# jhtonyKoo/music_mixing_style_transfer

Hardware: AMD Instinct MI355X
Metric: stereo 44.1 kHz segments/sec (FXencoder+MixFXcloner fwd) (higher is better)
Workload: dtype bf16

## Files before the change

### include/mst_hip.h

```cpp
#ifndef MST_HIP_H
#define MST_HIP_H

#include <stddef.h>
#include <stdint.h>

#ifdef __cplusplus
extern "C" {
#endif

typedef enum {
    MST_OK = 0,
    MST_ERR_ARG = -1,
    MST_ERR_UNSUPPORTED = -2,
    MST_ERR_HIP = -3,
    MST_ERR_STATE = -4,
    MST_ERR_WORKSPACE = -5
} MstStatus;

typedef enum {
    MST_PREC_F32 = 0,
    MST_PREC_BF16 = 1,
    MST_PREC_BF16X3 = 2
} MstPrecision;

#define MST_MAX_BLOCKS 32

int mst_version(void);
const char *mst_last_error(void);

typedef struct MstTcn MstTcn;

typedef struct {
    int nblocks;
    int ninputs;
    int noutputs;
    int channels;
    int kernel_size;
    int cond_dim;
    int dilations[MST_MAX_BLOCKS];
    int causal;
} MstTcnDesc;

int mst_tcn_create(const MstTcnDesc *desc, MstTcn **out);
int mst_tcn_destroy(MstTcn *tcn);

int mst_tcn_load_block(MstTcn *tcn, int n, const float *conv_w, const float *bn_weight, const float *bn_bias,
                       const float *bn_mean, const float *bn_var, float bn_eps, const float *film_w,
                       const float *film_b, const float *res_w, void *stream);
int mst_tcn_load_output(MstTcn *tcn, const float *w, const float *b, void *stream);

int mst_tcn_set_cond(MstTcn *tcn, const float *cond_dev, int n_rows, long block_stride, void *stream);

size_t mst_tcn_workspace_bytes(const MstTcn *tcn, int B, int L, int precision);

int mst_tcn_forward(MstTcn *tcn, const float *x_dev, float *y_dev, int B, int L, int precision,
                    void *workspace, size_t workspace_bytes, void *stream);
int mst_tcn_forward_blocks(MstTcn *tcn, const float *x_dev, float *act_dev, int B, int L, int precision, int n_run,
                           void *workspace, size_t workspace_bytes, void *stream);

int mst_tcn_set_tuning(MstTcn *tcn, int flags);
int mst_tcn_get_tuning(const MstTcn *tcn, int *flags, int *last_forward_fused_block0);

int mst_tcn_set_fusion(MstTcn *tcn, int flags);
int mst_tcn_get_fusion(const MstTcn *tcn, int *flags, int *last_forward_fused_tail);

int mst_tcn_context(const MstTcn *tcn, long *left, long *right);

int mst_tcn_timing_begin(MstTcn *tcn, int max_forwards);
int mst_tcn_timing_end(MstTcn *tcn, float *ms_out, int *n_forwards);

int mst_calib_mainloop(int launches, float *ms_per_launch, float *sclk_mhz, void *stream);

typedef struct MstEnc MstEnc;

typedef struct {
    int nblocks;
    int channels[MST_MAX_BLOCKS + 1];
    int kernels[MST_MAX_BLOCKS];
    int strides[MST_MAX_BLOCKS];
    int dilations[MST_MAX_BLOCKS];
    int valid_padding;
    float act_slope;
} MstEncDesc;

int mst_enc_create(const MstEncDesc *desc, MstEnc **out);
int mst_enc_destroy(MstEnc *enc);
int mst_enc_load_conv(MstEnc *enc, int block, int which, const float *w, const float *bias,
                      const float *bn_weight, const float *bn_bias, const float *bn_mean, const float *bn_var,
                      float bn_eps, void *stream);
int mst_enc_set_tuning(MstEnc *enc, long rows_min_tiles);
int mst_enc_set_schedule(MstEnc *enc, int flags);
int mst_global_avgpool(const float *x_dev, float *y_dev, long rows, int L, void *stream);
int mst_enc_zero_stuff(const float *x_dev, float *y_dev, long rows, long L, int stride, long pad_left, long Lu, void *stream);
size_t mst_enc_workspace_bytes(const MstEnc *enc, int B, int L);
int mst_enc_forward(MstEnc *enc, const float *x_dev, float *emb_dev, int B, int L, int precision, void *workspace,
                    size_t workspace_bytes, void *stream);
int mst_enc_forward_blocks(MstEnc *enc, const float *x_dev, float *out_dev, int B, int L, int precision, int n_run,
                           void *workspace, size_t workspace_bytes, void *stream);
int mst_enc_conv_length(const MstEnc *enc, int block, int which, int L);
int mst_enc_forward_conv(MstEnc *enc, int block, int which, const float *x_dev, float *y_dev, int B, int L, void *stream);
int mst_enc_block_length(const MstEnc *enc, int block, int L);

int mst_film_forward(const float *w_dev, const float *b_dev, const float *cond_dev, int rows, int cond_dim, int C,
                     const float *x_dev, float *y_dev, int B, long L, float *table_dev, void *stream);

int mst_embedding_mean(const float *emb_dev, int n_rows, int dim, float *out_dev, void *stream);

#define MST_SUMSQ_SLOTS 64
#define MST_FX_FORM_EQ_LANE_APPLY 1
#define MST_FX_FORM_EQ_VALU_ENDS 2
#define MST_FX_FORM_COMP_SLICE_SMALL 4
typedef struct {
    unsigned struct_size;
    int forms;
    const double *in_scale_dev;
    double *out_sumsq_dev;
    const double *in_sumsq_dev;
// ... 175 lines not shown
```

### music_mixing_style_transfer_amd/_lib.py

```python
import ctypes as C
import os

import torch

_HERE = os.path.dirname(os.path.abspath(__file__))
LIB_PATH = os.path.join(_HERE, "csrc", "libmst_hip.so")

MST_OK = 0
MST_PREC_F32 = 0
MST_PREC_BF16 = 1
MST_PREC_BF16X3 = 2
MST_MAX_BLOCKS = 32
TCN_TUNING_DEFAULT = 245
TCN_FUSION_DEFAULT = 1
PRECISIONS = {"fp32": MST_PREC_F32, "f32": MST_PREC_F32, "bf16": MST_PREC_BF16, "bf16x3": MST_PREC_BF16X3}

STATUS_NAMES = {0: "MST_OK", -1: "MST_ERR_ARG", -2: "MST_ERR_UNSUPPORTED", -3: "MST_ERR_HIP", -4: "MST_ERR_STATE",
                -5: "MST_ERR_WORKSPACE"}


class MstTcnDesc(C.Structure):
    _fields_ = [("nblocks", C.c_int), ("ninputs", C.c_int), ("noutputs", C.c_int), ("channels", C.c_int),
                ("kernel_size", C.c_int), ("cond_dim", C.c_int), ("dilations", C.c_int * MST_MAX_BLOCKS), ("causal", C.c_int)]


FX_FORM_EQ_LANE_APPLY, FX_FORM_EQ_VALU_ENDS, FX_FORM_COMP_SLICE_SMALL = 1, 2, 4


class MstFxFuse(C.Structure):
    _fields_ = [("struct_size", C.c_uint), ("forms", C.c_int), ("in_scale_dev", C.c_void_p), ("out_sumsq_dev", C.c_void_p),
                ("in_sumsq_dev", C.c_void_p), ("post_rms", C.c_int), ("post_gain", C.c_float), ("out_in_sumsq_dev", C.c_void_p),
                ("out_ms_dev", C.c_void_p), ("in_ms_dev", C.c_void_p)]

    def __init__(self, in_scale_dev=None, out_sumsq_dev=None, in_sumsq_dev=None, post_rms=0, post_gain=0.0, out_in_sumsq_dev=None,
                 out_ms_dev=None, in_ms_dev=None, forms=0):
        super().__init__(C.sizeof(MstFxFuse), forms, in_scale_dev, out_sumsq_dev, in_sumsq_dev, post_rms, post_gain, out_in_sumsq_dev,
                         out_ms_dev, in_ms_dev)


FX_COMP_SPLIT_SERIAL, FX_COMP_TIME_PARALLEL, FX_COMP_WAVE_SERIAL = 0, 1, 2


class MstFxBiquadItemsPlan(C.Structure):
    _fields_ = [("struct_size", C.c_uint), ("M", C.c_int), ("tables_offset", C.c_size_t), ("item_stride", C.c_size_t), ("powers_offset", C.c_size_t),
                ("coef_offset", C.c_size_t), ("total_bytes", C.c_size_t)]

    def __init__(self, *a, **kw):
        super().__init__(*a, **kw)
        self.struct_size = C.sizeof(MstFxBiquadItemsPlan)


class MstFxBiquadPlan(C.Structure):
    _fields_ = [("struct_size", C.c_uint), ("time_parallel", C.c_int), ("M", C.c_int), ("scan_threads", C.c_int), ("record_doubles", C.c_int),
                ("nchunks", C.c_long), ("ends_offset", C.c_size_t), ("starts_offset", C.c_size_t)]

    def __init__(self):
        super().__init__(C.sizeof(MstFxBiquadPlan))


class MstFxCompressorPlan(C.Structure):
    _fields_ = [("struct_size", C.c_uint), ("form", C.c_int), ("nslices", C.c_int), ("record_doubles", C.c_int), ("nchunks", C.c_long),
                ("nbatch", C.c_long), ("ntiles", C.c_long), ("kappa", C.c_double), ("kappa_limit", C.c_double), ("xl_offset", C.c_size_t),
                ("maps_offset", C.c_size_t), ("ystart_offset", C.c_size_t), ("tab_offset", C.c_size_t), ("carry_offset", C.c_size_t),
                ("tsums_offset", C.c_size_t), ("total_bytes", C.c_size_t)]

    def __init__(self):
        super().__init__(C.sizeof(MstFxCompressorPlan))


class MstEncDesc(C.Structure):
    _fields_ = [("nblocks", C.c_int), ("channels", C.c_int * (MST_MAX_BLOCKS + 1)), ("kernels", C.c_int * MST_MAX_BLOCKS),
                ("strides", C.c_int * MST_MAX_BLOCKS), ("dilations", C.c_int * MST_MAX_BLOCKS), ("valid_padding", C.c_int), ("act_slope", C.c_float)]


MST_MSS_MAX_SCALES = 8
MSS_MODES = {"midside": 0, "ori": 1}
MSS_WINDOWS = {"hann": 0, "hamming": 1}


class MstMssDesc(C.Structure):
    _fields_ = [("struct_size", C.c_uint), ("mode", C.c_int), ("n_scales", C.c_int), ("n_fft", C.c_int * MST_MSS_MAX_SCALES),
                ("hop", C.c_int * MST_MSS_MAX_SCALES), ("win_length", C.c_int * MST_MSS_MAX_SCALES), ("window", C.c_int),
                ("eps", C.c_double)]

    def __init__(self, mode=0, n_fft=(), hop=(), win_length=(), window=0, eps=1e-7):
        super().__init__()
        self.struct_size, self.mode, self.n_scales, self.window, self.eps = C.sizeof(MstMssDesc), mode, len(n_fft), window, eps
        for i in range(min(len(n_fft), MST_MSS_MAX_SCALES)):
            self.n_fft[i], self.hop[i], self.win_length[i] = n_fft[i], hop[i], win_length[i]


_P = C.c_void_p
_F = C.c_void_p

SIGNATURES = {
    "mst_version": (C.c_int, []),
    "mst_last_error": (C.c_char_p, []),
    "mst_tcn_create": (C.c_int, [C.POINTER(MstTcnDesc), C.POINTER(_P)]),
    "mst_tcn_destroy": (C.c_int, [_P]),
    "mst_tcn_load_block": (C.c_int, [_P, C.c_int, _F, _F, _F, _F, _F, C.c_float, _F, _F, _F, _P]),
    "mst_tcn_load_output": (C.c_int, [_P, _F, _F, _P]),
    "mst_tcn_set_cond": (C.c_int, [_P, _F, C.c_int, C.c_long, _P]),
    "mst_tcn_workspace_bytes": (C.c_size_t, [_P, C.c_int, C.c_int, C.c_int]),
    "mst_tcn_forward": (C.c_int, [_P, _F, _F, C.c_int, C.c_int, C.c_int, _P, C.c_size_t, _P]),
    "mst_tcn_forward_blocks": (C.c_int, [_P, _F, _F, C.c_int, C.c_int, C.c_int, C.c_int, _P, C.c_size_t, _P]),
    "mst_tcn_set_tuning": (C.c_int, [_P, C.c_int]),
    "mst_tcn_get_tuning": (C.c_int, [_P, C.POINTER(C.c_int), C.POINTER(C.c_int)]),
    "mst_tcn_set_fusion": (C.c_int, [_P, C.c_int]),
    "mst_tcn_get_fusion": (C.c_int, [_P, C.POINTER(C.c_int), C.POINTER(C.c_int)]),
    "mst_tcn_context": (C.c_int, [_P, C.POINTER(C.c_long), C.POINTER(C.c_long)]),
    "mst_tcn_timing_begin": (C.c_int, [_P, C.c_int]),
    "mst_tcn_timing_end": (C.c_int, [_P, C.POINTER(C.c_float), C.POINTER(C.c_int)]),
    "mst_calib_mainloop": (C.c_int, [C.c_int, C.POINTER(C.c_float), C.POINTER(C.c_float), _P]),
    "mst_enc_create": (C.c_int, [C.POINTER(MstEncDesc), C.POINTER(_P)]),
    "mst_enc_destroy": (C.c_int, [_P]),
    "mst_enc_load_conv": (C.c_int, [_P, C.c_int, C.c_int, _F, _F, _F, _F, _F, _F, C.c_float, _P]),
    "mst_enc_set_tuning": (C.c_int, [_P, C.c_long]),
    "mst_enc_set_schedule": (C.c_int, [_P, C.c_int]),
    "mst_global_avgpool": (C.c_int, [_F, _F, C.c_long, C.c_int, _P]),
    "mst_enc_zero_stuff": (C.c_int, [_F, _F, C.c_long, C.c_long, C.c_int, C.c_long, C.c_long, _P]),
    "mst_enc_workspace_bytes": (C.c_size_t, [_P, C.c_int, C.c_int]),
    "mst_enc_forward": (C.c_int, [_P, _F, _F, C.c_int, C.c_int, C.c_int, _P, C.c_size_t, _P]),
    "mst_enc_forward_blocks": (C.c_int, [_P, _F, _F, C.c_int, C.c_int, C.c_int, C.c_int, _P, C.c_size_t, _P]),
    "mst_enc_block_length": (C.c_int, [_P, C.c_int, C.c_int]),
    "mst_enc_conv_length": (C.c_int, [_P, C.c_int, C.c_int, C.c_int]),
    "mst_enc_forward_conv": (C.c_int, [_P, C.c_int, C.c_int, _F, _F, C.c_int, C.c_int, _P]),
    "mst_film_forward": (C.c_int, [_F, _F, _F, C.c_int, C.c_int, C.c_int, _F, _F, C.c_int, C.c_long, _F, _P]),
    "mst_embedding_mean": (C.c_int, [_F, C.c_int, C.c_int, _F, _P]),
    "mst_fx_biquad_scratch_bytes": (C.c_size_t, [C.c_int, C.c_long, C.c_int, C.c_int]),
    "mst_fx_biquad_plan": (C.c_int, [C.c_int, C.c_long, C.c_int, C.c_int, C.POINTER(MstFxBiquadPlan)]),
    "mst_fx_biquad_tables": (C.c_int, [C.POINTER(C.c_double), C.c_int, C.c_int, C.POINTER(C.c_double), C.POINTER(C.c_double)]),
    "mst_fx_compressor_plan": (C.c_int, [C.c_int, C.c_long, C.c_int, C.c_double, C.c_double, C.c_double, C.c_int, C.POINTER(MstFxCompressorPlan)]),
    "mst_fx_biquad_cascade": (C.c_int, [_F, _F, C.c_int, C.c_long, C.c_int, C.POINTER(C.c_double), C.c_int, _P, C.c_size_t, _P, _P]),
    "mst_fx_biquad_items_scratch_bytes": (C.c_size_t, [C.c_int, C.c_long, C.c_int, C.c_int]),
    "mst_fx_biquad_items_plan": (C.c_int, [C.c_int, C.c_long, C.c_int, C.c_int, C.POINTER(MstFxBiquadItemsPlan)]),
    "mst_fx_biquad_cascade_items": (C.c_int, [_F, _F, C.c_int, C.c_long, C.c_int, _P, C.c_int, _P, C.c_size_t, _P, _P]),
    "mst_fx_compressor_items_table_bytes": (C.c_size_t, [C.c_int]),
    "mst_fx_compressor_items_prepare": (C.c_int, [_P, C.c_int, C.c_long, C.c_int, C.c_double, C.c_int, _P, C.c_size_t, C.POINTER(C.c_int)]),
    "mst_fx_compressor_items": (C.c_int, [_F, _F, C.c_int, C.c_long, C.c_int, _P, _P, C.c_size_t, _P, _P]),
    "mst_fx_midside_imager_items": (C.c_int, [_F, _F, C.c_int, C.c_long, _P, _P, _P, _P, _P]),
    "mst_fx_gain_items": (C.c_int, [_F, _F, C.c_int, C.c_long, C.c_int, _P, _P, _P, _P]),
    "mst_fx_sumsq": (C.c_int, [_F, C.c_int, C.c_long, _P, _P]),
    "mst_fx_rms_pending": (C.c_int, [_P, _P, C.c_long, _P, C.c_long, _P, C.c_int, _P]),
    "mst_fx_scale_items": (C.c_int, [_F, _F, C.c_int, C.c_long, _P, _P]),
    "mst_fx_compressor_scratch_bytes": (C.c_size_t, [C.c_int, C.c_long, C.c_int]),
    "mst_fx_compressor": (C.c_int, [_F, _F, C.c_int, C.c_long, C.c_int, C.c_double, C.c_double, C.c_double, C.c_double,
                                    C.c_double, _P, C.c_size_t, _P, _P]),
    "mst_fx_midside_imager": (C.c_int, [_F, _F, C.c_int, C.c_long, C.c_double, _P, _P, _P]),
    "mst_fx_gain": (C.c_int, [_F, _F, C.c_int, C.c_long, C.c_int, C.c_double, C.c_int, _P, _P]),
    "mst_fx_haas": (C.c_int, [_F, _F, C.c_int, C.c_long, C.c_int, C.c_long, C.c_double, C.c_int, _P]),
    "mst_fx_panner": (C.c_int, [_F, _F, C.c_int, C.c_long, C.c_int, C.c_float, C.c_float, _P]),
    "mst_fx_rms_normalize": (C.c_int, [_F, _F, C.c_int, C.c_long, C.c_long, _P, _P]),
    "mst_fx_convolver_create": (C.c_int, [C.c_long, C.c_long, C.c_int, C.c_int, C.POINTER(_P)]),
    "mst_fx_convolver_destroy": (None, [_P]),
    "mst_fx_convolver_workspace_bytes": (C.c_size_t, [_P]),
    "mst_fx_compressor_grid": (C.c_int, [_F, _F, C.c_int, C.c_long, C.c_int, _F, _F, C.c_double, C.c_double, C.c_double, _P, C.c_size_t,
                                         _P, _P]),
    "mst_fx_range_reduce": (C.c_int, [_F, C.c_long, C.c_int, C.c_int, _P, _P, _P, C.c_int, C.c_int, _P, _P]),
    "mst_fx_onset_hfc": (C.c_int, [_F, C.c_int, C.c_long, C.c_int, C.c_int, C.c_int, _F, _P]),
    "mst_fx_stft_create": (C.c_int, [C.c_long, C.c_long, C.POINTER(C.c_float), C.c_int, C.POINTER(_P)]),
    "mst_fx_stft_destroy": (None, [_P]),
    "mst_fx_stft_workspace_bytes": (C.c_size_t, [_P]),
# ... 109 lines not shown
```

### music_mixing_style_transfer_amd/csrc/mst_api.hip

```cpp
#include "mst_host.h"

namespace {
thread_local std::string g_err;
}

int mst_fail(int code, const std::string &msg) {
    g_err = msg;
    return code;
}

extern "C" int mst_version(void) { return 109; }
extern "C" const char *mst_last_error(void) { return g_err.c_str(); }
```

### music_mixing_style_transfer_amd/csrc/mst_tcn.hip

```cpp
#include "mst_host.h"
#include "tcn_kernels.h"

struct MstTcnBlock {
    void *w_bf16 = nullptr;
    void *w_x3 = nullptr;
    float *w_f32 = nullptr;
    float *shift = nullptr;
    float *res = nullptr;
    bool loaded = false;
};

struct TcnTuning {
    int flags;
    bool x3_small_tiles() const { return flags & 1; }
    bool bf16_cm() const { return ((flags >> 1) & 3) == 2; }
    bool bf16_fuse0() const { return bf16_cm() && (flags & 32); }
    bool x3_half_cm() const { return flags & 64; }
    bool bf16_whole() const { return bf16_cm() && (flags & 128); }
};

constexpr int TCN_FILM_ROWS0 = 64;
struct MstTcn {
    MstTcnDesc d;
    bool generic = false;
    std::vector<MstEncConv> gconv;
    std::vector<MstTcnBlock> blk;
    float *film_w = nullptr;
    float *film_b = nullptr;
    float *film = nullptr;
    int film_rows = 0, film_cap = 0;
    std::vector<float *> film_retired;
    float *out_w = nullptr, *out_b = nullptr;
    bool out_loaded = false;
    void *zero_row = nullptr;
    int tuning = 245;
    int last_fused0 = 0;
    int fusion = 0;
    int last_fused_tail = 0;
    std::vector<hipEvent_t> ev;
    std::vector<char> ev_tail;
    int ev_max = 0, ev_used = 0;
};


extern "C" int mst_tcn_create(const MstTcnDesc *desc, MstTcn **out) {
    if (!desc || !out) return fail(MST_ERR_ARG, "mst_tcn_create: null argument");
    const MstTcnDesc &d = *desc;
    if (d.nblocks < 1 || d.nblocks > MST_MAX_BLOCKS) return fail(MST_ERR_ARG, "mst_tcn_create: nblocks out of range");
    if (d.channels < 1 || d.kernel_size < 1 || d.ninputs < 1 || d.noutputs < 1 || d.cond_dim < 1)
        return fail(MST_ERR_ARG, "mst_tcn_create: bad layer description");
    if (d.channels % d.ninputs != 0)
        return fail(MST_ERR_UNSUPPORTED, "mst_tcn_create: channel_width must be a multiple of ninputs (grouped 1x1 residual)");
    const bool fast = d.channels == 128 && d.kernel_size == 15 && d.ninputs == 2 && d.noutputs <= 2 && d.dilations[0] == 1 && !d.causal;
    for (int n = 0; n < d.nblocks; ++n)
        if (d.dilations[n] < 1) return fail(MST_ERR_ARG, "mst_tcn_create: dilation < 1");
    MstTcn *t = new MstTcn();
    t->d = d;
    t->generic = !fast;
    t->blk.resize(d.nblocks);
    if (t->generic) {
        t->gconv.resize(d.nblocks + 1);
        for (int n = 0; n < d.nblocks; ++n) {
            const int span = (d.kernel_size - 1) * d.dilations[n];
            const int pad_l = d.causal ? span : span / 2;
            conv_geometry(t->gconv[n], n == 0 ? d.ninputs : d.channels, d.channels, d.kernel_size, 1, d.dilations[n], pad_l, span - pad_l);
        }
        conv_geometry(t->gconv[d.nblocks], d.channels, d.noutputs, 1, 1, 1, 0, 0);
    }
    const size_t fw = (size_t)d.nblocks * 2 * d.channels * d.cond_dim;
    if (hipMalloc((void **)&t->film_w, fw * sizeof(float)) != hipSuccess ||
        hipMalloc((void **)&t->film_b, (size_t)d.nblocks * 2 * d.channels * sizeof(float)) != hipSuccess ||
        hipMalloc(&t->zero_row, 1024) != hipSuccess || hipMemset(t->zero_row, 0, 1024) != hipSuccess ||
        hipMalloc((void **)&t->film, (size_t)d.nblocks * TCN_FILM_ROWS0 * 2 * d.channels * sizeof(float)) != hipSuccess) {
        (void)hipFree(t->film_w);
        (void)hipFree(t->film_b);
        (void)hipFree(t->zero_row);
        (void)hipFree(t->film);
        delete t;
        return fail(MST_ERR_HIP, "mst_tcn_create: hipMalloc failed");
    }
    t->film_cap = TCN_FILM_ROWS0;
    *out = t;
    return MST_OK;
}

extern "C" int mst_tcn_destroy(MstTcn *t) {
    if (!t) return MST_OK;
    for (auto &b : t->blk) {
        (void)hipFree(b.w_bf16);
        (void)hipFree(b.w_x3);
        (void)hipFree(b.w_f32);
        (void)hipFree(b.shift);
        (void)hipFree(b.res);
    }
    (void)hipFree(t->film_w);
    (void)hipFree(t->film_b);
    (void)hipFree(t->film);
    for (float *f : t->film_retired) (void)hipFree(f);
    (void)hipFree(t->out_w);
    (void)hipFree(t->out_b);
    (void)hipFree(t->zero_row);
    for (auto &c : t->gconv) {
        (void)hipFree(c.wpk);
        (void)hipFree(c.ktab);
        (void)hipFree(c.shift);
    }
    for (auto e : t->ev) (void)hipEventDestroy(e);
    delete t;
    return MST_OK;
}

extern "C" int mst_tcn_load_block(MstTcn *t, int n, const float *conv_w, const float *bn_weight, const float *bn_bias,
                                  const float *bn_mean, const float *bn_var, float bn_eps, const float *film_w,
                                  const float *film_b, const float *res_w, void *) {
    if (!t || !conv_w || !bn_weight || !bn_bias || !bn_mean || !bn_var || !film_w || !film_b || !res_w)
        return fail(MST_ERR_ARG, "mst_tcn_load_block: null argument");
    if (n < 0 || n >= t->d.nblocks) return fail(MST_ERR_ARG, "mst_tcn_load_block: block index out of range");
    const int C = t->d.channels, K = t->d.kernel_size;
    const int cin = n == 0 ? t->d.ninputs : C;
    std::vector<float> scale, shift;
    bn_fold(bn_weight, bn_bias, bn_mean, bn_var, bn_eps, C, scale, shift);
    MstTcnBlock &b = t->blk[n];
    auto W = [&](int co, int ci, int j) { return conv_w[((size_t)co * cin + ci) * K + j] * scale[co]; };
    int rc;
    if (t->generic) {
        MstEncConv &c = t->gconv[n];
        if ((rc = pack_conv_f32(c, conv_w, scale))) return rc;
        std::vector<float> sh((size_t)((C + 32 * c.mw - 1) / (32 * c.mw)) * 32 * c.mw, 0.0f);
        for (int co = 0; co < C; ++co) sh[co] = shift[co];
        if ((rc = upload(&c.shift, sh))) return rc;
        c.loaded = true;
    } else if (n == 0) {
        std::vector<float> w0((size_t)cin * K * C);
        for (int ci = 0; ci < cin; ++ci)
            for (int j = 0; j < K; ++j)
                for (int co = 0; co < C; ++co) w0[((size_t)ci * K + j) * C + co] = W(co, ci, j);
        if ((rc = upload(&b.w_f32, w0))) return rc;
        std::vector<__bf16> wb((size_t)2 * 4 * 64 * 8);
        for (int sI = 0; sI < 2; ++sI)
            for (int w = 0; w < 4; ++w)
                for (int l = 0; l < 64; ++l)
                    for (int e = 0; e < 8; ++e) {
                        const int k = 16 * sI + 8 * (l >> 5) + e;
                        wb[(((size_t)sI * 4 + w) * 64 + l) * 8 + e] = k < 30 ? (__bf16)W(32 * w + (l & 31), k / 15, k % 15) : (__bf16)0.0f;
                    }
        if ((rc = upload((__bf16 **)&b.w_bf16, wb))) return rc;
    } else {
        const size_t image = (size_t)120 * 4 * 64 * 8;
        std::vector<__bf16> wb(image), wx(2 * image);
        for (int j = 0; j < K; ++j)
            for (int kk = 0; kk < 4; ++kk)
                for (int m = 0; m < 2; ++m)
                    for (int w = 0; w < 4; ++w)
                        for (int l = 0; l < 64; ++l)
                            for (int e = 0; e < 8; ++e) {
                                const float v = W(32 * w + 16 * m + (l & 15), 32 * kk + 8 * (l >> 4) + e, j);
                                const __bf16 hi = (__bf16)v;
                                const size_t idx = (((((size_t)(j * 4 + kk) * 2 + m) * 4 + w) * 64 + l) * 8) + e;
                                wb[idx] = wx[idx] = hi;
                                wx[image + idx] = (__bf16)(v - (float)hi);
// ... 177 lines not shown
    TCN_BF16_KERNEL(8,  false, 4, 0, false),
    TCN_BF16_KERNEL(8,  true,  4, 0, false),
    TCN_BF16_KERNEL(8,  false, 4, 1, false),
    TCN_BF16_KERNEL(8,  true,  4, 1, false),
    TCN_X3_KERNEL(1, 8),
    TCN_X3_KERNEL(2, 8),
    TCN_X3_KERNEL(4, 8),
    TCN_X3_KERNEL(1, 4),
    TCN_X3_KERNEL(2, 4),
    TCN_X3_HALF_KERNEL(8, 4, false),
    TCN_X3_HALF_KERNEL(8, 4, true),
    TCN_F32_KERNEL(1),
    TCN_F32_KERNEL(2),
    TCN_F32_KERNEL(4),
    TCN_F32_KERNEL(8),
    TCN_F32_KERNEL(16),
};
#undef TCN_BF16_KERNEL
#undef TCN_X3_KERNEL
#undef TCN_X3_HALF_KERNEL
#undef TCN_F32_KERNEL

int tcn_launch_block(const TcnBlockPlan &p, const TcnBlockArgs &a, void *stream) {
    for (const TcnBlockKernel &k : TCN_BLOCK_KERNELS)
        if (k.family == p.family && k.P == p.P && k.tile == p.tile && k.form == p.form && k.block0 == p.block0 &&
            (k.head == p.head || p.family != TCN_BF16)) {
            MST_LAUNCH(k.kernel, dim3((unsigned)p.grid), dim3(256), stream, a);
            MST_CHECK_LAUNCH(k.name);
            return MST_OK;
        }
    return fail(MST_ERR_STATE, "mst_tcn_forward: no block kernel of this tile form (with the fused head the whole-sequence 256-time tile exists at "
                               "sixteen phases only)");
}

int tcn_run_generic(MstTcn *t, const float *x, float *y, float *act_out, int B, int L, int n_run, void *ws, void *stream) {
    const int C = t->d.channels;
    const size_t buf_bytes = align_up((size_t)B * L * C * sizeof(float), 256);
    float *buf[2] = {(float *)ws, (float *)((unsigned char *)ws + buf_bytes)};
    const float *cur = x;
    int rc, pp = 0;
    for (int n = 0; n < n_run; ++n) {
        float *dst = (act_out && n == n_run - 1) ? act_out : buf[pp];
        const int cin = n == 0 ? t->d.ninputs : C;
        if ((rc = tcn_launch_generic(t->gconv[n], cur, dst, B, L, 1, t->film + (size_t)n * t->film_rows * 2 * C, t->film_rows,
                                     t->blk[n].res, C / cin, stream)))
            return rc;
        cur = dst;
        pp ^= 1;
    }
    if (act_out) return MST_OK;
    return tcn_launch_generic(t->gconv[t->d.nblocks], cur, y, B, L, 2, nullptr, 1, nullptr, 1, stream);
}

int tcn_run(MstTcn *t, const float *x, float *y, float *act_out, int B, int L, int precision, int n_run, void *ws,
            size_t ws_bytes, void *stream) {
    if (!t || !x || B < 1 || L < 1) return fail(MST_ERR_ARG, "mst_tcn_forward: bad argument");
    if (precision != MST_PREC_F32 && precision != MST_PREC_BF16 && precision != MST_PREC_BF16X3)
        return fail(MST_ERR_ARG, "mst_tcn_forward: bad precision");
    for (auto &b : t->blk)
        if (!b.loaded) return fail(MST_ERR_STATE, "mst_tcn_forward: block weights not loaded");
    if (!t->out_loaded) return fail(MST_ERR_STATE, "mst_tcn_forward: output conv not loaded");
    if (t->film_rows == 0) return fail(MST_ERR_STATE, "mst_tcn_forward: mst_tcn_set_cond has not been called");
    if (t->film_rows != 1 && t->film_rows != B)
        return fail(MST_ERR_ARG, "mst_tcn_forward: condition rows must be 1 or equal the batch size");
    const size_t need = mst_tcn_workspace_bytes(t, B, L, precision);
    if (!ws || ws_bytes < need) return fail(MST_ERR_WORKSPACE, "mst_tcn_forward: workspace too small");
    if (t->generic) return tcn_run_generic(t, x, y, act_out, B, L, n_run, ws, stream);
    const int nblocks = t->d.nblocks;
    TcnBlockPlan plan[MST_MAX_BLOCKS] = {};
    for (int n = 1; n < n_run; ++n) {
        plan[n] = tcn_plan_block(t->tuning, precision, t->d.dilations[n], L, B, !act_out && n == nblocks - 1,
                                 n == 1 && nblocks > 2 && t->d.dilations[0] == 1);
        if (plan[n].grid > 0x7fffffffL) return fail(MST_ERR_ARG, "mst_tcn_forward: grid too large");
    }
    bool tail = false;
    if (precision == MST_PREC_BF16 && !act_out && n_run == nblocks && nblocks >= 4 && (t->fusion & 1)) {
        const int n0 = nblocks - 3;
        const int d0 = t->d.dilations[n0];
        tail = t->d.dilations[n0 + 1] == 2 * d0 && t->d.dilations[n0 + 2] == 4 * d0;
        for (int k = 0; k < 3; ++k) {
            const TcnBlockPlan &p = plan[n0 + k];
            tail = tail && p.family == TCN_BF16 && p.form == 1 && p.tile == 256 && p.P == (4 << k) && p.tiles_step == 1 && !p.block0 &&
                   p.head == (k == 2) && p.grid == plan[n0].grid;
        }
    }
    t->last_fused_tail = tail ? 1 : 0;
    const size_t buf_bytes = align_up((size_t)B * L * 128 * tcn_elem(precision), 256);
    unsigned char *buf[2] = {(unsigned char *)ws, (unsigned char *)ws + buf_bytes};
    const int Lp = L;
    hipEvent_t *ev = nullptr;
    if (!act_out && t->ev_used < t->ev_max) {
        ev = t->ev.data() + (size_t)t->ev_used * (nblocks + 2);
        t->ev_tail[t->ev_used] = tail ? 1 : 0;
        t->ev_used++;
        MST_HIP_TRY(hipEventRecord(ev[0], (hipStream_t)stream));
    }

    const bool fuse0 = plan[1].block0;
    t->last_fused0 = fuse0 ? 1 : 0;
    if (!fuse0) {
        TcnBlock0Args a;
        a.x = x;
        a.y = buf[0];
        a.w = t->blk[0].w_f32;
        a.shift = t->blk[0].shift;
        a.film = t->film;
        a.res = t->blk[0].res;
        a.film_rows = t->film_rows;
        a.B = B;
        a.L = L;
        a.Lp = Lp;
        a.wpk16 = t->blk[0].w_bf16;
        if (precision == MST_PREC_BF16)
            MST_LAUNCH(tcn_block0_mfma_kernel, dim3(B * ((L + 255) / 256)), dim3(256), stream, a);
        else
            MST_LAUNCH((tcn_block0_kernel<float>), dim3(B * ((L + 511) / 512)), dim3(256), stream, a);
        MST_CHECK_LAUNCH("tcn_block0_kernel");
    }
    if (ev) MST_HIP_TRY(hipEventRecord(ev[1], (hipStream_t)stream));
    int cur = 0;
    for (int n = 1; n < n_run; ++n) {
        const TcnBlockPlan &p = plan[n];
        TcnBlockArgs a;
        a.x = buf[cur];
        a.y = buf[cur ^ 1];
        a.wpk = precision == MST_PREC_BF16 ? t->blk[n].w_bf16 : (precision == MST_PREC_BF16X3 ? t->blk[n].w_x3 : (void *)t->blk[n].w_f32);
        a.shift = t->blk[n].shift;
        a.film = t->film + (size_t)n * t->film_rows * 256;
        a.res = t->blk[n].res;
        a.film_rows = t->film_rows;
        a.B = B;
        a.L = L;
        a.Lp = Lp;
        a.d = t->d.dilations[n];
        a.tiles_phase = p.tiles_phase;
        a.tiles_step = p.tiles_step;
        a.out_w = t->out_w;
        a.out_b = t->out_b;
        a.y_out = p.head ? y : nullptr;
        a.nout = t->d.noutputs;
        a.xcd_tiles = p.xcd_tiles;
        a.zeros = t->zero_row;
        if (p.block0) {
            a.x0 = x;
            a.w0pk = t->blk[0].w_bf16;
            a.shift0 = t->blk[0].shift;
            a.film0 = t->film;
            a.res0 = t->blk[0].res;
        }
        if (tail && n == nblocks - 3) {
            TcnTailArgs ta;
            ta.a = a;
            ta.a.y = nullptr;
            ta.a.y_out = y;
            for (int k = 0; k < 3; ++k) {
                ta.wpk[k] = t->blk[n + k].w_bf16;
                ta.shift[k] = t->blk[n + k].shift;
                ta.film[k] = t->film + (size_t)(n + k) * t->film_rows * 256;
                ta.res[k] = t->blk[n + k].res;
            }
            MST_LAUNCH(tcn_tail_bf16_kernel, dim3((unsigned)p.grid), dim3(256), stream, ta);
            MST_CHECK_LAUNCH("tcn_tail_bf16_kernel");
            if (ev)
                for (int k = 0; k < 3; ++k) MST_HIP_TRY(hipEventRecord(ev[n + k + 1], (hipStream_t)stream));
            break;
        }
        int rc;
        if ((rc = tcn_launch_block(p, a, stream))) return rc;
        if (ev) MST_HIP_TRY(hipEventRecord(ev[n + 1], (hipStream_t)stream));
        cur ^= 1;
    }
    if (act_out) {
        const size_t total = (size_t)B * L * 128;
        const unsigned grid = (unsigned)((total + 255) / 256);
        if (precision == MST_PREC_BF16)
            MST_LAUNCH((tcn_unpack_kernel<__bf16>), dim3(grid), dim3(256), stream, (const void *)buf[cur], act_out, B, L, Lp);
        else
            MST_LAUNCH((tcn_unpack_kernel<float>), dim3(grid), dim3(256), stream, (const void *)buf[cur], act_out, B, L, Lp);
        MST_CHECK_LAUNCH("tcn_unpack_kernel");
        return MST_OK;
    }
    if (!plan[nblocks - 1].head) {
        TcnOutArgs o;
        o.x = buf[cur];
        o.y = y;
        o.w = t->out_w;
        o.bias = t->out_b;
        o.nout = t->d.noutputs;
        o.B = B;
        o.L = L;
        o.Lp = Lp;
        const int grid = B * ((L + 63) / 64);
        if (precision == MST_PREC_BF16)
            MST_LAUNCH((tcn_output_kernel<__bf16>), dim3(grid), dim3(256), stream, o);
        else
            MST_LAUNCH((tcn_output_kernel<float>), dim3(grid), dim3(256), stream, o);
        MST_CHECK_LAUNCH("tcn_output_kernel");
    }
    if (ev) MST_HIP_TRY(hipEventRecord(ev[nblocks + 1], (hipStream_t)stream));
    return MST_OK;
}

}

extern "C" int mst_tcn_set_tuning(MstTcn *t, int flags) {
    if (!t) return fail(MST_ERR_ARG, "mst_tcn_set_tuning: null handle");
    const int form = (flags >> 1) & 3;
    if (flags < 0 || flags > 255 || (form != 0 && form != 2) || ((flags >> 3) & 1) || (form == 2 && !((flags >> 4) & 1)))
        return fail(MST_ERR_ARG, "mst_tcn_set_tuning: unknown flag bits (bits 1-2 = 0 or 2, form 2 with bit 4, no bit 3: the kernels the others "
                                 "selected left the library)");
    t->tuning = flags;
    return MST_OK;
}

extern "C" int mst_tcn_get_tuning(const MstTcn *t, int *flags, int *last_forward_fused_block0) {
    if (!t) return fail(MST_ERR_ARG, "mst_tcn_get_tuning: null handle");
    if (flags) *flags = t->tuning;
    if (last_forward_fused_block0) *last_forward_fused_block0 = t->last_fused0;
    return MST_OK;
}

extern "C" int mst_tcn_set_fusion(MstTcn *t, int flags) {
    if (!t) return fail(MST_ERR_ARG, "mst_tcn_set_fusion: null handle");
    if (flags < 0 || flags > 1) return fail(MST_ERR_ARG, "mst_tcn_set_fusion: unknown flag bits (bit 0: the last three blocks as one launch)");
    t->fusion = flags;
    return MST_OK;
}

extern "C" int mst_tcn_get_fusion(const MstTcn *t, int *flags, int *last_forward_fused_tail) {
    if (!t) return fail(MST_ERR_ARG, "mst_tcn_get_fusion: null handle");
    if (flags) *flags = t->fusion;
    if (last_forward_fused_tail) *last_forward_fused_tail = t->last_fused_tail;
    return MST_OK;
}

extern "C" int mst_tcn_context(const MstTcn *t, long *left, long *right) {
    if (!t) return fail(MST_ERR_ARG, "mst_tcn_context: null handle");
    long l = 0, r = 0;
    for (int n = 0; n < t->d.nblocks; ++n) {
        const long span = (long)(t->d.kernel_size - 1) * t->d.dilations[n];
        const long pad_l = t->d.causal ? span : span / 2;
        l += pad_l;
        r += span - pad_l;
    }
    if (left) *left = l;
    if (right) *right = r;
    return MST_OK;
}

extern "C" int mst_tcn_timing_begin(MstTcn *t, int max_forwards) {
    if (!t || max_forwards < 1) return fail(MST_ERR_ARG, "mst_tcn_timing_begin: bad argument");
    for (auto e : t->ev) (void)hipEventDestroy(e);
    t->ev.assign((size_t)max_forwards * (t->d.nblocks + 2), nullptr);
    for (auto &e : t->ev) MST_HIP_TRY(hipEventCreate(&e));
    t->ev_tail.assign((size_t)max_forwards, 0);
    t->ev_max = max_forwards;
    t->ev_used = 0;
    return MST_OK;
}

extern "C" int mst_tcn_timing_end(MstTcn *t, float *ms_out, int *n_forwards) {
    if (!t || !ms_out || !n_forwards) return fail(MST_ERR_ARG, "mst_tcn_timing_end: bad argument");
    const int per = t->d.nblocks + 2;
    for (int k = 0; k <= t->d.nblocks; ++k) ms_out[k] = 0.0f;
    for (int f = 0; f < t->ev_used; ++f) {
        MST_HIP_TRY(hipEventSynchronize(t->ev[(size_t)f * per + per - 1]));
        float ms[MST_MAX_BLOCKS + 1] = {};
        for (int k = 0; k <= t->d.nblocks; ++k) MST_HIP_TRY(hipEventElapsedTime(&ms[k], t->ev[(size_t)f * per + k], t->ev[(size_t)f * per + k + 1]));
        if (t->ev_tail[f]) {
            const int n0 = t->d.nblocks - 3;
            ms[n0] = ms[n0 + 1] = ms[n0 + 2] = (ms[n0] + ms[n0 + 1] + ms[n0 + 2]) / 3.0f;
        }
        for (int k = 0; k <= t->d.nblocks; ++k) ms_out[k] += ms[k];
    }
    if (t->ev_used > 0)
        for (int k = 0; k <= t->d.nblocks; ++k) ms_out[k] /= (float)t->ev_used;
    *n_forwards = t->ev_used;
    for (auto e : t->ev) (void)hipEventDestroy(e);
    t->ev.clear();
    t->ev_max = t->ev_used = 0;
    return MST_OK;
}

extern "C" int mst_calib_mainloop(int launches, float *ms_per_launch, float *sclk_mhz, void *stream) {
    if (launches < 2 || !ms_per_launch || !sclk_mhz) return fail(MST_ERR_ARG, "mst_calib_mainloop: bad argument");
    constexpr int WG = 512, REP = 32;
    const size_t wbytes = (size_t)120 * 256 * 16;
    void *w = nullptr;
    float *out = nullptr;
    long long *clk = nullptr;
    hipEvent_t e0 = nullptr, e1 = nullptr;
    int rc = MST_OK;
    auto cleanup = [&]() {
        if (w) (void)hipFree(w);
        if (out) (void)hipFree(out);
        if (clk) (void)hipFree(clk);
        if (e0) (void)hipEventDestroy(e0);
        if (e1) (void)hipEventDestroy(e1);
    };
#define MST_CALIB_TRY(x)                                                        \
    if ((x) != hipSuccess) {                                                    \
        rc = fail(MST_ERR_HIP, "mst_calib_mainloop: HIP call failed");          \
        cleanup();                                                              \
        return rc;                                                              \
    }
    MST_CALIB_TRY(hipMalloc(&w, wbytes));
    MST_CALIB_TRY(hipMalloc((void **)&out, (size_t)WG * 256 * sizeof(float)));
    MST_CALIB_TRY(hipMalloc((void **)&clk, 2 * sizeof(long long)));
    MST_CALIB_TRY(hipEventCreate(&e0));
    MST_CALIB_TRY(hipEventCreate(&e1));
    MST_LAUNCH(tcn_calib_fill_kernel, dim3((unsigned)(wbytes / 4 + 255) / 256), dim3(256), stream, (unsigned *)w, (int)(wbytes / 4));
    const int warm = launches / 2, timed = launches - warm;
    for (int i = 0; i < warm; ++i) MST_LAUNCH(tcn_calib_mainloop_kernel, dim3(WG), dim3(256), stream, (const void *)w, out, clk, REP);
    MST_CALIB_TRY(hipEventRecord(e0, (hipStream_t)stream));
    for (int i = 0; i < timed; ++i) MST_LAUNCH(tcn_calib_mainloop_kernel, dim3(WG), dim3(256), stream, (const void *)w, out, clk, REP);
    MST_CALIB_TRY(hipEventRecord(e1, (hipStream_t)stream));
    MST_CALIB_TRY(hipEventSynchronize(e1));
    float ms = 0.0f;
    MST_CALIB_TRY(hipEventElapsedTime(&ms, e0, e1));
    long long c[2] = {0, 0};
    MST_CALIB_TRY(hipMemcpy(c, clk, sizeof(c), hipMemcpyDeviceToHost));
#undef MST_CALIB_TRY
    *ms_per_launch = ms / (float)timed;
    *sclk_mhz = c[1] > 0 ? (float)((double)c[0] / ((double)c[1] / 100.0)) : 0.0f;
    cleanup();
    return MST_OK;
}

extern "C" size_t mst_tcn_workspace_bytes(const MstTcn *t, int B, int L, int precision) {
    if (B < 1 || L < 1) return 0;
    if (t && t->generic) return 2 * align_up((size_t)B * L * t->d.channels * sizeof(float), 256);
    return 2 * align_up((size_t)B * L * 128 * tcn_elem(precision), 256);
}
// ... 37 lines not shown
```

### music_mixing_style_transfer_amd/networks/architectures.py

```python
import ctypes as C
import inspect
import os

import torch
import torch.nn as nn

from .. import _lib
from .network_utils import Conv1d_layer, ConvBlock, FiLM, Res_ConvBlock, _DeviceState


class _HParams(dict):

    def __getattr__(self, k):
        try:
            return self[k]
        except KeyError:
            raise AttributeError(k) from None

    def __setattr__(self, k, v):
        self[k] = v


def _stream_ptr(t):
    return _lib.lib().stream_ptr(t)
# ... 274 lines not shown
                                        grouped=grouped, conditional=True if nparams > 0 else False))
        self.output = nn.Conv1d(out_ch, noutputs, kernel_size=1)
        self.precision = os.environ.get("MST_TCN_PRECISION", "fp32")
        self._handle = None
        self._lib = None
        self._sig = None
        self._ws = _Workspace()

    def compute_receptive_field(self):
        hp = self.hparams
        rf = hp.kernel_size
        for n in range(1, hp.nblocks):
            rf += (hp.kernel_size - 1) * hp.dilation_growth ** (n % hp.stack_size)
        return rf

    def context(self):
        hp = self.hparams
        left = right = 0
        for blk in self.blocks:
            span = (hp.kernel_size - 1) * blk.dilation
            pad_l = span if hp.causal else span // 2
            left, right = left + pad_l, right + span - pad_l
        return left, right

    @staticmethod
    def add_model_specific_args(parent_parser):
        from argparse import ArgumentParser
        parser = ArgumentParser(parents=[parent_parser], add_help=False)
        for name, default in (("ninputs", 1), ("noutputs", 1), ("nblocks", 4), ("kernel_size", 5), ("dilation_growth", 10),
                              ("channel_growth", 1), ("channel_width", 32), ("stack_size", 10)):
            parser.add_argument("--" + name, type=int, default=default)
        for name in ("grouped", "causal", "skip_connections"):
            parser.add_argument("--" + name, default=False, action="store_true")
        return parser

    def _ensure(self, b):
        sig = _signature(self)
        if self._handle is not None and sig == self._sig and self._lib is b:
            return
        self._close()
        hp = self.hparams
        if not hp.nparams > 0:
            raise AttributeError("'TCNBlock' object has no attribute 'film'")
        d = _lib.MstTcnDesc()
        held = list(self.blocks)[-1:] if hp.channel_growth > 1 else list(self.blocks)
        d.nblocks, d.ninputs, d.noutputs = len(held), held[0].in_ch, hp.noutputs
        d.channels, d.kernel_size, d.cond_dim, d.causal = held[-1].out_ch, hp.kernel_size, hp.cond_dim, int(bool(hp.causal))
        for n, blk in enumerate(held):
            d.dilations[n] = blk.dilation
        h = C.c_void_p()
        b.check(b.mst_tcn_create(C.byref(d), C.byref(h)), "mst_tcn_create")
        self._handle, self._lib = h, b
        b.check(b.mst_tcn_set_fusion(h, _lib.TCN_FUSION_DEFAULT), "mst_tcn_set_fusion")
        f = lambda t: t.detach().to("cpu", torch.float32).contiguous()
        for n, blk in enumerate(held):
            _load_tcn_block(b, h, n, blk)
        ow, ob = f(self.output.weight), f(self.output.bias)
        b.check(b.mst_tcn_load_output(h, ow.data_ptr(), ob.data_ptr(), None), "mst_tcn_load_output")
        self._sig = sig

    def _close(self):
        if self._handle is not None:
            self._lib.mst_tcn_destroy(self._handle)
            self._handle = None

    def __del__(self):
        try:
            self._close()
        except Exception:
            pass

    def _set_cond(self, b, x, cond):
        hp = self.hparams
        if isinstance(cond, (list, tuple)):
            if len(cond) != hp.nblocks:
                raise ValueError("TCNModel.forward: a condition list needs one entry per block")
            if hp.channel_growth > 1:
                cond = cond[-1:]
            c = torch.stack([ci.to(x.device, torch.float32) for ci in cond], 0).contiguous()
            rows, stride = c.shape[1], c.shape[1] * c.shape[2]
        else:
            c = cond.to(x.device, torch.float32).contiguous()
            rows, stride = c.shape[0], 0
        if c.shape[-1] != hp.cond_dim:
            raise ValueError(f"TCNModel.forward: condition length {c.shape[-1]} != cond_dim {hp.cond_dim}")
        if rows not in (1, x.shape[0]):
            raise RuntimeError(f"The size of tensor a ({rows}) must match the size of tensor b ({x.shape[0]}) at "
                               f"non-singleton dimension 0")
        b.check(b.mst_tcn_set_cond(self._handle, c.data_ptr(), rows, stride, _stream_ptr(x)), "mst_tcn_set_cond")
        return c

    def forward(self, x, cond):
        return self._run(x, cond, None)

    def forward_blocks(self, x, cond, n_run):
        return self._run(x, cond, n_run)

    def _run(self, x, cond, n_run):
        b = _check_device(x, "TCNModel.forward")
        with b.device_ctx(x):
            return self._run_on(b, x, cond, n_run)

    def _run_on(self, b, x, cond, n_run):
        hp = self.hparams
        if x.dim() != 3 or x.shape[1] != hp.ninputs:
            raise ValueError(f"TCNModel.forward: expected [B, {hp.ninputs}, L], got {tuple(x.shape)}")
# ... 28 lines not shown
```

Baseline: 1823.

## Split TCN batch into cache-sized chunks run on two alternating streams

Adds batch chunking to the TCN forward so each chunk's ping-pong activation buffers fit in a roughly 256 MB cache budget. Chunks alternate between the main stream and a pooled side stream, joined by events, so two chains can overlap. The Python wrapper turns on automatic chunking by default. This adds more kernel launches and some stream and event overhead, and changes how per-block timing is collected.

Result: faster. 1884, median of 6 (+3.4%).

```diff
diff --git a/include/mst_hip.h b/include/mst_hip.h
--- a/include/mst_hip.h
+++ b/include/mst_hip.h
@@ -63,6 +63,10 @@
 
 int mst_tcn_set_fusion(MstTcn *tcn, int flags);
 int mst_tcn_get_fusion(const MstTcn *tcn, int *flags, int *last_forward_fused_tail);
+
+#define MST_TCN_CHUNK_WHOLE 0x7fffffff
+int mst_tcn_set_chunk(MstTcn *tcn, int items);
+int mst_tcn_get_chunk(const MstTcn *tcn, int *items, int *ran_chunks);
 
 int mst_tcn_context(const MstTcn *tcn, long *left, long *right);
 
diff --git a/music_mixing_style_transfer_amd/_lib.py b/music_mixing_style_transfer_amd/_lib.py
--- a/music_mixing_style_transfer_amd/_lib.py
+++ b/music_mixing_style_transfer_amd/_lib.py
@@ -13,6 +13,8 @@
 MST_MAX_BLOCKS = 32
 TCN_TUNING_DEFAULT = 245
 TCN_FUSION_DEFAULT = 1
+TCN_CHUNK_DEFAULT = 0
+TCN_CHUNK_WHOLE = 0x7fffffff
 PRECISIONS = {"fp32": MST_PREC_F32, "f32": MST_PREC_F32, "bf16": MST_PREC_BF16, "bf16x3": MST_PREC_BF16X3}
 
 STATUS_NAMES = {0: "MST_OK", -1: "MST_ERR_ARG", -2: "MST_ERR_UNSUPPORTED", -3: "MST_ERR_HIP", -4: "MST_ERR_STATE",
@@ -108,6 +110,8 @@
     "mst_tcn_get_tuning": (C.c_int, [_P, C.POINTER(C.c_int), C.POINTER(C.c_int)]),
     "mst_tcn_set_fusion": (C.c_int, [_P, C.c_int]),
     "mst_tcn_get_fusion": (C.c_int, [_P, C.POINTER(C.c_int), C.POINTER(C.c_int)]),
+    "mst_tcn_set_chunk": (C.c_int, [_P, C.c_int]),
+    "mst_tcn_get_chunk": (C.c_int, [_P, C.POINTER(C.c_int), C.POINTER(C.c_int)]),
     "mst_tcn_context": (C.c_int, [_P, C.POINTER(C.c_long), C.POINTER(C.c_long)]),
     "mst_tcn_timing_begin": (C.c_int, [_P, C.c_int]),
     "mst_tcn_timing_end": (C.c_int, [_P, C.POINTER(C.c_float), C.POINTER(C.c_int)]),
diff --git a/music_mixing_style_transfer_amd/csrc/mst_api.hip b/music_mixing_style_transfer_amd/csrc/mst_api.hip
--- a/music_mixing_style_transfer_amd/csrc/mst_api.hip
+++ b/music_mixing_style_transfer_amd/csrc/mst_api.hip
@@ -9,5 +9,5 @@
     return code;
 }
 
-extern "C" int mst_version(void) { return 109; }
+extern "C" int mst_version(void) { return 110; }
 extern "C" const char *mst_last_error(void) { return g_err.c_str(); }
diff --git a/music_mixing_style_transfer_amd/csrc/mst_tcn.hip b/music_mixing_style_transfer_amd/csrc/mst_tcn.hip
--- a/music_mixing_style_transfer_amd/csrc/mst_tcn.hip
+++ b/music_mixing_style_transfer_amd/csrc/mst_tcn.hip
@@ -37,10 +37,24 @@
     int last_fused0 = 0;
     int fusion = 0;
     int last_fused_tail = 0;
+    int chunk = MST_TCN_CHUNK_WHOLE;
+    int last_chunks = 1;
+    hipStream_t side = nullptr;
+    hipEvent_t side_fork = nullptr, side_join = nullptr;
+    int side_dev = -1;
     std::vector<hipEvent_t> ev;
-    std::vector<char> ev_tail;
-    int ev_max = 0, ev_used = 0;
+    struct TimedForward {
+        size_t first;
+        int chunks, chains;
+        bool tail;
+    };
+    std::vector<TimedForward> ev_fwd;
+    size_t ev_next = 0;
+    int ev_max = 0;
 };
+
+static std::mutex tcn_side_mu;
+static std::vector<std::pair<int, hipStream_t>> tcn_side_free;
 
 
 extern "C" int mst_tcn_create(const MstTcnDesc *desc, MstTcn **out) {
@@ -106,6 +120,12 @@
         (void)hipFree(c.shift);
     }
     for (auto e : t->ev) (void)hipEventDestroy(e);
+    if (t->side_fork) (void)hipEventDestroy(t->side_fork);
+    if (t->side_join) (void)hipEventDestroy(t->side_join);
+    if (t->side_dev >= 0) {
+        std::lock_guard<std::mutex> lock(tcn_side_mu);
+        tcn_side_free.emplace_back(t->side_dev, t->side);
+    }
     delete t;
     return MST_OK;
 }
@@ -389,20 +409,8 @@
     return tcn_launch_generic(t->gconv[t->d.nblocks], cur, y, B, L, 2, nullptr, 1, nullptr, 1, stream);
 }
 
-int tcn_run(MstTcn *t, const float *x, float *y, float *act_out, int B, int L, int precision, int n_run, void *ws,
-            size_t ws_bytes, void *stream) {
-    if (!t || !x || B < 1 || L < 1) return fail(MST_ERR_ARG, "mst_tcn_forward: bad argument");
-    if (precision != MST_PREC_F32 && precision != MST_PREC_BF16 && precision != MST_PREC_BF16X3)
-        return fail(MST_ERR_ARG, "mst_tcn_forward: bad precision");
-    for (auto &b : t->blk)
-        if (!b.loaded) return fail(MST_ERR_STATE, "mst_tcn_forward: block weights not loaded");
-    if (!t->out_loaded) return fail(MST_ERR_STATE, "mst_tcn_forward: output conv not loaded");
-    if (t->film_rows == 0) return fail(MST_ERR_STATE, "mst_tcn_forward: mst_tcn_set_cond has not been called");
-    if (t->film_rows != 1 && t->film_rows != B)
-        return fail(MST_ERR_ARG, "mst_tcn_forward: condition rows must be 1 or equal the batch size");
-    const size_t need = mst_tcn_workspace_bytes(t, B, L, precision);
-    if (!ws || ws_bytes < need) return fail(MST_ERR_WORKSPACE, "mst_tcn_forward: workspace too small");
-    if (t->generic) return tcn_run_generic(t, x, y, act_out, B, L, n_run, ws, stream);
+int tcn_run_items(MstTcn *t, const float *x, float *y, float *act_out, int B, int L, int precision, int n_run, unsigned char *buf0,
+                  unsigned char *buf1, size_t film_row0, hipEvent_t *ev, void *stream) {
     const int nblocks = t->d.nblocks;
     TcnBlockPlan plan[MST_MAX_BLOCKS] = {};
     for (int n = 1; n < n_run; ++n) {
@@ -422,16 +430,10 @@
         }
     }
     t->last_fused_tail = tail ? 1 : 0;
-    const size_t buf_bytes = align_up((size_t)B * L * 128 * tcn_elem(precision), 256);
-    unsigned char *buf[2] = {(unsigned char *)ws, (unsigned char *)ws + buf_bytes};
+    unsigned char *buf[2] = {buf0, buf1};
     const int Lp = L;
-    hipEvent_t *ev = nullptr;
-    if (!act_out && t->ev_used < t->ev_max) {
-        ev = t->ev.data() + (size_t)t->ev_used * (nblocks + 2);
-        t->ev_tail[t->ev_used] = tail ? 1 : 0;
-        t->ev_used++;
-        MST_HIP_TRY(hipEventRecord(ev[0], (hipStream_t)stream));
-    }
+    const float *film = t->film + film_row0 * 256;
+    if (ev) MST_HIP_TRY(hipEventRecord(ev[0], (hipStream_t)stream));
 
     const bool fuse0 = plan[1].block0;
     t->last_fused0 = fuse0 ? 1 : 0;
@@ -441,7 +443,7 @@
         a.y = buf[0];
         a.w = t->blk[0].w_f32;
         a.shift = t->blk[0].shift;
-        a.film = t->film;
+        a.film = film;
         a.res = t->blk[0].res;
         a.film_rows = t->film_rows;
         a.B = B;
@@ -463,7 +465,7 @@
         a.y = buf[cur ^ 1];
         a.wpk = precision == MST_PREC_BF16 ? t->blk[n].w_bf16 : (precision == MST_PREC_BF16X3 ? t->blk[n].w_x3 : (void *)t->blk[n].w_f32);
         a.shift = t->blk[n].shift;
-        a.film = t->film + (size_t)n * t->film_rows * 256;
+        a.film = film + (size_t)n * t->film_rows * 256;
         a.res = t->blk[n].res;
         a.film_rows = t->film_rows;
         a.B = B;
@@ -482,7 +484,7 @@
             a.x0 = x;
             a.w0pk = t->blk[0].w_bf16;
             a.shift0 = t->blk[0].shift;
-            a.film0 = t->film;
+            a.film0 = film;
             a.res0 = t->blk[0].res;
         }
         if (tail && n == nblocks - 3) {
@@ -493,7 +495,7 @@
             for (int k = 0; k < 3; ++k) {
                 ta.wpk[k] = t->blk[n + k].w_bf16;
                 ta.shift[k] = t->blk[n + k].shift;
-                ta.film[k] = t->film + (size_t)(n + k) * t->film_rows * 256;
+                ta.film[k] = film + (size_t)(n + k) * t->film_rows * 256;
                 ta.res[k] = t->blk[n + k].res;
             }
             MST_LAUNCH(tcn_tail_bf16_kernel, dim3((unsigned)p.grid), dim3(256), stream, ta);
@@ -538,6 +540,95 @@
     return MST_OK;
 }
 
+constexpr size_t TCN_CACHE_BYTES = (size_t)256 << 20;
+constexpr int TCN_CHUNK_CHAINS = 2;
+
+int tcn_chunk_items(int B, int L) {
+    const size_t item = (size_t)L * 128 * 2;
+    if ((size_t)B * item <= TCN_CACHE_BYTES) return B;
+    const size_t c = TCN_CACHE_BYTES / (2 * TCN_CHUNK_CHAINS * item);
+    return c >= 1 ? (int)c : B;
+}
+
+int tcn_side_stream(MstTcn *t) {
+    const int dev = mst_current_device();
+    if (t->side_dev >= 0 && t->side_dev != dev) return fail(MST_ERR_STATE, "mst_tcn_forward: the handle's side stream lives on another device");
+    if (t->side_dev >= 0) return MST_OK;
+    if (!t->side_fork) MST_HIP_TRY(hipEventCreateWithFlags(&t->side_fork, hipEventDisableTiming));
+    if (!t->side_join) MST_HIP_TRY(hipEventCreateWithFlags(&t->side_join, hipEventDisableTiming));
+    {
+        std::lock_guard<std::mutex> lock(tcn_side_mu);
+        for (size_t i = 0; i < tcn_side_free.size(); ++i)
+            if (tcn_side_free[i].first == dev) {
+                t->side = tcn_side_free[i].second;
+                t->side_dev = dev;
+                tcn_side_free.erase(tcn_side_free.begin() + i);
+                return MST_OK;
+            }
+    }
+    MST_HIP_TRY(hipStreamCreateWithPriority(&t->side, hipStreamNonBlocking, 0));
+    t->side_dev = dev;
+    return MST_OK;
+}
+
+int tcn_run(MstTcn *t, const float *x, float *y, float *act_out, int B, int L, int precision, int n_run, void *ws,
+            size_t ws_bytes, void *stream) {
+    if (!t || !x || B < 1 || L < 1) return fail(MST_ERR_ARG, "mst_tcn_forward: bad argument");
+    if (precision != MST_PREC_F32 && precision != MST_PREC_BF16 && precision != MST_PREC_BF16X3)
+        return fail(MST_ERR_ARG, "mst_tcn_forward: bad precision");
+    for (auto &b : t->blk)
+        if (!b.loaded) return fail(MST_ERR_STATE, "mst_tcn_forward: block weights not loaded");
+    if (!t->out_loaded) return fail(MST_ERR_STATE, "mst_tcn_forward: output conv not loaded");
+    if (t->film_rows == 0) return fail(MST_ERR_STATE, "mst_tcn_forward: mst_tcn_set_cond has not been called");
+    if (t->film_rows != 1 && t->film_rows != B)
+        return fail(MST_ERR_ARG, "mst_tcn_forward: condition rows must be 1 or equal the batch size");
+    const size_t need = mst_tcn_workspace_bytes(t, B, L, precision);
+    if (!ws || ws_bytes < need) return fail(MST_ERR_WORKSPACE, "mst_tcn_forward: workspace too small");
+    t->last_chunks = 1;
+    if (t->generic) return tcn_run_generic(t, x, y, act_out, B, L, n_run, ws, stream);
+    const int nblocks = t->d.nblocks;
+    const int per = nblocks + 2;
+    int c = B;
+    if (precision == MST_PREC_BF16 && !act_out && n_run == nblocks && nblocks >= 2) c = std::min(B, t->chunk > 0 ? t->chunk : tcn_chunk_items(B, L));
+    const int chunks = (B + c - 1) / c;
+    const size_t buf_bytes = align_up((size_t)c * L * 128 * tcn_elem(precision), 256);
+    const int chains = chunks >= 2 && 2 * TCN_CHUNK_CHAINS * buf_bytes <= need ? TCN_CHUNK_CHAINS : 1;
+    int rc;
+    if (chains > 1 && (rc = tcn_side_stream(t))) return rc;
+    hipEvent_t *ev = nullptr;
+    if (!act_out && (int)t->ev_fwd.size() < t->ev_max) {
+        while (t->ev.size() < t->ev_next + (size_t)chunks * per) {
+            hipEvent_t e = nullptr;
+            MST_HIP_TRY(hipEventCreate(&e));
+            t->ev.push_back(e);
+        }
+        ev = t->ev.data() + t->ev_next;
+        t->ev_fwd.push_back({t->ev_next, chunks, chains, false});
+        t->ev_next += (size_t)chunks * per;
+    }
+    if (chains > 1) {
+        MST_HIP_TRY(hipEventRecord(t->side_fork, (hipStream_t)stream));
+        MST_HIP_TRY(hipStreamWaitEvent(t->side, t->side_fork, 0));
+    }
+    rc = MST_OK;
+    for (int k = 0; k < chunks && rc == MST_OK; ++k) {
+        const int b0 = k * c, nb = std::min(c, B - b0);
+        const int chain = k % chains;
+        unsigned char *base = (unsigned char *)ws + (size_t)chain * 2 * buf_bytes;
+        rc = tcn_run_items(t, x + (size_t)b0 * t->d.ninputs * L, y ? y + (size_t)b0 * t->d.noutputs * L : nullptr, act_out, nb, L, precision, n_run,
+                           base, base + buf_bytes, t->film_rows > 1 ? (size_t)b0 : 0, ev ? ev + (size_t)k * per : nullptr,
+                           chain ? (void *)t->side : stream);
+    }
+    if (chains > 1) {
+        hipError_t e = hipEventRecord(t->side_join, t->side);
+        if (e == hipSuccess) e = hipStreamWaitEvent((hipStream_t)stream, t->side_join, 0);
+        if (e != hipSuccess && rc == MST_OK) rc = fail(MST_ERR_HIP, std::string("mst_tcn_forward: joining the side stream: ") + hipGetErrorString(e));
+    }
+    if (ev) t->ev_fwd.back().tail = t->last_fused_tail != 0;
+    t->last_chunks = chunks;
+    return rc;
+}
+
 }
 
 extern "C" int mst_tcn_set_tuning(MstTcn *t, int flags) {
@@ -568,6 +659,20 @@
     if (!t) return fail(MST_ERR_ARG, "mst_tcn_get_fusion: null handle");
     if (flags) *flags = t->fusion;
     if (last_forward_fused_tail) *last_forward_fused_tail = t->last_fused_tail;
+    return MST_OK;
+}
+
+extern "C" int mst_tcn_set_chunk(MstTcn *t, int items) {
+    if (!t) return fail(MST_ERR_ARG, "mst_tcn_set_chunk: null handle");
+    if (items < 0) return fail(MST_ERR_ARG, "mst_tcn_set_chunk: items < 0 (0: automatic, n: n items per chunk, MST_TCN_CHUNK_WHOLE: never)");
+    t->chunk = items;
+    return MST_OK;
+}
+
+extern "C" int mst_tcn_get_chunk(const MstTcn *t, int *items, int *ran_chunks) {
+    if (!t) return fail(MST_ERR_ARG, "mst_tcn_get_chunk: null handle");
+    if (items) *items = t->chunk;
+    if (ran_chunks) *ran_chunks = t->last_chunks;
     return MST_OK;
 }
 
@@ -590,9 +695,10 @@
     for (auto e : t->ev) (void)hipEventDestroy(e);
     t->ev.assign((size_t)max_forwards * (t->d.nblocks + 2), nullptr);
     for (auto &e : t->ev) MST_HIP_TRY(hipEventCreate(&e));
-    t->ev_tail.assign((size_t)max_forwards, 0);
+    t->ev_fwd.clear();
+    t->ev_fwd.reserve((size_t)max_forwards);
     t->ev_max = max_forwards;
-    t->ev_used = 0;
+    t->ev_next = 0;
     return MST_OK;
 }
 
@@ -600,22 +706,27 @@
     if (!t || !ms_out || !n_forwards) return fail(MST_ERR_ARG, "mst_tcn_timing_end: bad argument");
     const int per = t->d.nblocks + 2;
     for (int k = 0; k <= t->d.nblocks; ++k) ms_out[k] = 0.0f;
-    for (int f = 0; f < t->ev_used; ++f) {
-        MST_HIP_TRY(hipEventSynchronize(t->ev[(size_t)f * per + per - 1]));
-        float ms[MST_MAX_BLOCKS + 1] = {};
-        for (int k = 0; k <= t->d.nblocks; ++k) MST_HIP_TRY(hipEventElapsedTime(&ms[k], t->ev[(size_t)f * per + k], t->ev[(size_t)f * per + k + 1]));
-        if (t->ev_tail[f]) {
-            const int n0 = t->d.nblocks - 3;
-            ms[n0] = ms[n0 + 1] = ms[n0 + 2] = (ms[n0] + ms[n0 + 1] + ms[n0 + 2]) / 3.0f;
-        }
-        for (int k = 0; k <= t->d.nblocks; ++k) ms_out[k] += ms[k];
-    }
-    if (t->ev_used > 0)
-        for (int k = 0; k <= t->d.nblocks; ++k) ms_out[k] /= (float)t->ev_used;
-    *n_forwards = t->ev_used;
+    const int used = (int)t->ev_fwd.size();
+    for (const MstTcn::TimedForward &f : t->ev_fwd)
+        for (int c = 0; c < f.chunks; ++c) {
+            const hipEvent_t *ev = t->ev.data() + f.first + (size_t)c * per;
+            MST_HIP_TRY(hipEventSynchronize(ev[per - 1]));
+            float ms[MST_MAX_BLOCKS + 1] = {};
+            for (int k = 0; k <= t->d.nblocks; ++k) MST_HIP_TRY(hipEventElapsedTime(&ms[k], ev[k], ev[k + 1]));
+            if (f.tail) {
+                const int n0 = t->d.nblocks - 3;
+                ms[n0] = ms[n0 + 1] = ms[n0 + 2] = (ms[n0] + ms[n0 + 1] + ms[n0 + 2]) / 3.0f;
+            }
+            for (int k = 0; k <= t->d.nblocks; ++k) ms_out[k] += ms[k] / (float)f.chains;
+        }
+    if (used > 0)
+        for (int k = 0; k <= t->d.nblocks; ++k) ms_out[k] /= (float)used;
+    *n_forwards = used;
     for (auto e : t->ev) (void)hipEventDestroy(e);
     t->ev.clear();
-    t->ev_max = t->ev_used = 0;
+    t->ev_fwd.clear();
+    t->ev_max = 0;
+    t->ev_next = 0;
     return MST_OK;
 }
 
diff --git a/music_mixing_style_transfer_amd/networks/architectures.py b/music_mixing_style_transfer_amd/networks/architectures.py
--- a/music_mixing_style_transfer_amd/networks/architectures.py
+++ b/music_mixing_style_transfer_amd/networks/architectures.py
@@ -350,6 +350,7 @@
         b.check(b.mst_tcn_create(C.byref(d), C.byref(h)), "mst_tcn_create")
         self._handle, self._lib = h, b
         b.check(b.mst_tcn_set_fusion(h, _lib.TCN_FUSION_DEFAULT), "mst_tcn_set_fusion")
+        b.check(b.mst_tcn_set_chunk(h, _lib.TCN_CHUNK_DEFAULT), "mst_tcn_set_chunk")
         f = lambda t: t.detach().to("cpu", torch.float32).contiguous()
         for n, blk in enumerate(held):
             _load_tcn_block(b, h, n, blk)
```
